# LanaSina/evolutionary_illusion_generator

Measured on AMD Instinct MI355X. Metric: genome fitness evals/sec at 256x256, pop=256, higher is better.
Workload: dtype f32; 1 GPU; neat_configs/circles.txt colour pop=256, 256x256, PredNet 3,48,96,192, 21 steps, LK + rotation-symmetry score; global_pop=256, genomes_per_gpu=256, device_batch=256, structure=Circles

## Files before the change

evolutionary_illusion_generator_amd/csrc/conv_wino4.h:

```cpp
#pragma once
#include "wino_launch.h"

namespace eig {

constexpr int W4_UPOS = 256;
constexpr int W4_U_FLOATS = W4_NPOS * W4_UPOS;
constexpr int W4_NUS = 3, W4_NPS = 3;
constexpr int w4_row(bool tall) { return tall ? 28 : 40; }
constexpr int w4_ps(bool tall) { return tall ? 1024 : 768; }
constexpr int w4_pslot(bool tall) { return W4_KC * w4_ps(tall); }
constexpr int w4_p(bool tall, int k) { return tall ? k * w4_pslot(true) : (k < 2 ? k * w4_pslot(false) : 2 * w4_pslot(false) + 3 * W4_U_FLOATS); }
constexpr int w4_u(bool tall, int k) { return tall ? 3 * w4_pslot(true) + k * W4_U_FLOATS : 2 * w4_pslot(false) + k * W4_U_FLOATS; }
constexpr int w4_x(bool tall) { return tall ? w4_u(true, 0) : w4_u(false, 1); }
constexpr int W4_X_FLOATS = W4_WAVES * 2 * 4 * 64 * 4;
constexpr int wino4_lds_bytes() { return (w4_x(false) + W4_X_FLOATS) * 4; }
static_assert((w4_u(true, 2) + W4_U_FLOATS) * 4 == wino4_lds_bytes() && (w4_p(false, 2) + w4_pslot(false)) * 4 <= wino4_lds_bytes(), "LDS maps");
#ifndef EIG_W4_DEEPU
#define EIG_W4_DEEPU 1
#endif
#ifndef EIG_W4_DIAG
#define EIG_W4_DIAG 0
#endif

__device__ __forceinline__ void w4_in1d(float d0, float d1, float d2, float d3, float d4, float d5, float* T)
{
    T[0] = fmaf(4.0f, d0, fmaf(-5.0f, d2, d4));
    const float p = fmaf(-4.0f, d2, d4), q = fmaf(-4.0f, d1, d3);
    T[1] = p + q; T[2] = p - q;
    const float r = d4 - d2, s = d3 - d1;
    T[3] = fmaf(2.0f, s, r); T[4] = fmaf(-2.0f, s, r);
    T[5] = fmaf(4.0f, d1, fmaf(-5.0f, d3, d5));
}
template <int XI> __device__ __forceinline__ float w4_row(const float* d)
{
    if constexpr (XI == 0) return fmaf(4.0f, d[0], fmaf(-5.0f, d[1], d[2]));
    else if constexpr (XI == 5) return fmaf(4.0f, d[0], fmaf(-5.0f, d[1], d[2]));
    else {
        if constexpr (XI == 1) return fmaf(-4.0f, d[1], d[3]) + fmaf(-4.0f, d[0], d[2]);
        else if constexpr (XI == 2) return fmaf(-4.0f, d[1], d[3]) - fmaf(-4.0f, d[0], d[2]);
        else if constexpr (XI == 3) return fmaf(2.0f, d[2] - d[0], d[3] - d[1]);
        else return fmaf(-2.0f, d[2] - d[0], d[3] - d[1]);
    }
}
constexpr int w4_nrows(int xi) { return (xi == 0 || xi == 5) ? 3 : 4; }
constexpr int w4_rowidx(int xi, int k) { return xi == 0 ? 2 * k : xi == 5 ? 2 * k + 1 : k + 1; }
constexpr int w4_uprow(int i) { return (i + 1) >> 1; }

template <typename V4> __device__ __forceinline__ void w4_out1d(const V4& m0, const V4& m1, const V4& m2, const V4& m3, const V4& m4, const V4& m5, V4* Y)
{
    const V4 s = m1 + m2, d = m1 - m2, u = m3 + m4, w = m3 - m4;
    Y[0] = (m0 + s) + u;
    for (int e = 0; e < 4; ++e) { Y[1][e] = fmaf(2.0f, w[e], d[e]); Y[2][e] = fmaf(4.0f, u[e], s[e]); Y[3][e] = fmaf(8.0f, w[e], d[e]) + m5[e]; }
}

template <int NI, int EPI, bool TALL = false, bool HALF = false, bool PACK = false, bool NSPLIT = false>
__global__ void __launch_bounds__((HALF && !NSPLIT) ? W4_THREADS / 2 : W4_THREADS, 3) wino4_kernel(const ConvArgs a)
{
    static_assert(!NSPLIT || (HALF && NI == 4 && EPI != EPI_CONVA), "N-split: a half block, 64-column N-blocks, ConvLSTM / ConvP");
    constexpr int NIW = NSPLIT ? 2 : NI;
    constexpr bool DEEPU = HALF && EIG_W4_DEEPU;
    static_assert(!(TALL && HALF), "half blocks exist in the wide shape only");
    static_assert(!PACK || (HALF && EPI != EPI_CONVA), "packed tiles: a half block, ConvLSTM / ConvP");
    constexpr bool TGEO = TALL || PACK;
    static_assert(EPI == EPI_LSTM || EPI == EPI_CONVA || EPI == EPI_CONVP, "conv_wino4.h: ConvLSTM, ConvA, ConvP");
    static_assert(EPI != EPI_LSTM || NI == 4, "ConvLSTM: the four N-tiles are the four gates");
    static_assert(NI == 3 || NI == 4, "N-blocks of 48 or 64 columns");
    constexpr int U4 = wino4_u_floats(NI);
    constexpr int KC = W4_KC, PS = w4_ps(TGEO), W4_ROW = w4_row(TGEO);
    constexpr int W4_P0 = w4_p(TGEO, 0), W4_P1 = w4_p(TGEO, 1), W4_P2 = w4_p(TGEO, 2), W4_U0 = w4_u(TGEO, 0), W4_U1 = w4_u(TGEO, 1), W4_U2 = w4_u(TGEO, 2);
    constexpr int PK_ROWS = 18, PK_CX = 7, PK_IMG = PK_ROWS * PK_CX;
    constexpr bool WALK = !TALL && !HALF;
    constexpr int RGH = TALL ? 16 : 8;
    extern __shared__ __attribute__((aligned(16))) float lds[];
    unsigned long long tq_entry = EIG_TIMING ? __builtin_readcyclecounter() : 0;
    float* const Pb = lds;
    float* const Ub = lds;
    float* const xb = lds + w4_x(TGEO);
    const int wv_o = __builtin_amdgcn_readfirstlane((int)threadIdx.x >> 6);
    const int rg_o = HALF ? 0 : wv_o & 1, xi_o = (HALF && !NSPLIT) ? wv_o : wv_o >> 1;
    const int ng_o = NSPLIT ? wv_o & 1 : 0;
    constexpr int NWAVES = (HALF && !NSPLIT) ? W4_WAVES / 2 : W4_WAVES;
    constexpr int UPW = 36 / NWAVES;
    auto lane_id = [&]() __attribute__((always_inline)) { int l = (int)__builtin_amdgcn_mbcnt_hi(~0u, __builtin_amdgcn_mbcnt_lo(~0u, 0u)); asm volatile("" : "+v"(l)); return l; };

    const int tiles = a.tilesX * a.tilesY;
    const bool pk5 = PACK && a.tilesX == 5;
    const int ntile = PACK ? a.B + (pk5 ? (a.B + 3) >> 2 : 0) : a.B * tiles;
    const int xcd = blockIdx.x & 7, xi_ = blockIdx.x >> 3;
    auto dv = [&](int x, int d, unsigned m) __attribute__((always_inline)) { return m ? (int)__umulhi((unsigned)x, m) : x / d; };
    const int q0 = dv(xi_, a.nparts, a.mg[0]);
    const int part = xi_ - q0 * a.nparts;
    const int tlin = a.tile_map ? xcd * ((ntile + 7) >> 3) + q0 : q0 * 8 + xcd;
    if (tlin >= ntile) return;
    const int nwalk = WALK ? a.nwalk : 1, nb0 = part * nwalk;
    const bool pk_edge_o = pk5 && tlin >= a.B;
    const int eb = PACK ? (pk_edge_o ? 4 * (tlin - a.B) : tlin) : dv(tlin, tiles, a.mg[1]);
    const int t_ = PACK ? 0 : tlin - eb * tiles;
    const int tyi = dv(t_, a.tilesX, a.mg[2]), txi = t_ - tyi * a.tilesX;
    const int y0 = PACK ? 0 : tyi * (TALL ? 32 : (HALF ? 8 : 16)), x0 = PACK ? 0 : txi * (TALL ? 16 : 32);
    const int HW = a.H * a.W;

    const bool up_fused = !PACK && EPI == EPI_LSTM && a.up_src != nullptr;
    const int nkb0 = a.src[0].C / KC;
    const int nkbu = up_fused ? (a.up_C / KC) : 0;
    const bool has1 = a.nsrc > 1;
    const int nkb_o = nkb0 + nkbu + (has1 ? (a.src[1].C / KC) : 0);
    const int up_lo_o = nkb0, up_hi_o = nkb0 + nkbu;
#define EIG4_WAITCNT(imm) do { __builtin_amdgcn_s_waitcnt(imm); asm volatile("" ::: "memory"); } while (0)
#define EIG4_BARRIER() do { asm volatile("" ::: "memory"); __builtin_amdgcn_s_barrier(); asm volatile("" ::: "memory"); } while (0)
#define EIG4_LDS_BARRIER() do { EIG4_WAITCNT(0xC07F); EIG4_BARRIER(); } while (0)
#define EIG4_IS_UP(kb) ((kb) >= up_lo && (kb) < up_hi)

    typedef float f32x2 __attribute__((ext_vector_type(2)));
    constexpr unsigned W4_POSB = 4 * 16 * NI * 4;
    auto walk_body = [&](const int it) __attribute__((always_inline)) {
    const int nblk = nb0 + it;
    int zs = 0;
    asm volatile("" : "+s"(zs));
    const int wv = wv_o + zs, rg = rg_o + zs, xi = xi_o + zs, ng = ng_o + zs, nkb = nkb_o + zs, up_lo = up_lo_o + zs, up_hi = up_hi_o + zs;
    const int pch = HALF ? wv >> 1 : wv / 3, ppart = HALF ? wv & 1 : wv - pch * 3;
    const bool has_plane = !(NSPLIT && !PACK) || wv_o < 8;
    const int eb_i = eb + zs, y0_i = y0 + zs, x0_i = x0 + zs;
    const bool pk_edge = (pk_edge_o ? 1 : 0) + zs != 0;
    const unsigned long long sb0 = (unsigned long long)(a.src[0].ptr + (size_t)eb_i * a.src[0].Ct * HW);
    const unsigned long long sb1 = has1 ? (unsigned long long)(a.src[1].ptr + (size_t)eb_i * a.src[1].Ct * HW) : sb0;
    const int ist0 = a.src[0].Ct * HW * 4, ist1 = has1 ? a.src[1].Ct * HW * 4 : ist0;
    const int sz0 = a.src[0].C * HW * 4 + (PACK ? 3 * ist0 : 0), sz1 = has1 ? a.src[1].C * HW * 4 + (PACK ? 3 * ist1 : 0) : sz0;
    const int Hh = a.H >> 1, Wh = a.W >> 1, HWh = Hh * Wh;
    const unsigned long long sbu = up_fused ? (unsigned long long)(a.up_src + (size_t)eb_i * a.up_C * HWh) : sb0;
    const int szu = up_fused ? a.up_C * HWh * 4 : sz0;
    const int lane = lane_id();
    const int q = lane >> 4, col = lane & 15;
    constexpr int CPR = TALL ? 7 : 10, CREAL = TALL ? 6 : 10, NCHK = TALL ? 34 * 7 : (HALF ? 100 : 180), UROWS = TALL ? 18 : (HALF ? 6 : 10), UCHK = TALL ? 4 : 6;
    auto plane_offsets = [&](int part, int& ro, int& uo) __attribute__((always_inline)) {
        const int c = lane + 64 * part;
        const int row = c / CPR, cx = c - row * CPR;
        const int gy = y0_i - 1 + row, gx = x0_i - 4 + 4 * cx;
        ro = (c < NCHK && cx < CREAL && gy >= 0 && gy < a.H && gx >= 0 && gx < a.W) ? (gy * a.W + gx) * 4 : -1;
        const int hy = (y0_i >> 1) - 1 + row, hx = (x0_i >> 1) - 4 + 4 * cx;
        uo = (row < UROWS && cx < UCHK && hy >= 0 && hy < Hh && hx >= 0 && hx < Wh) ? (hy * Wh + hx) * 4 : -1;
    };
    int pk_ro[3] = {-1, -1, -1};
    unsigned pk_mul[3] = {0u, 0u, 0u};
    const int pk_n = (wv_o < 4 ? 2 : 1) + (NSPLIT ? 0 : 1);
    if constexpr (PACK) {
#pragma unroll
        for (int k = 0; k < 3; ++k) {
            const int c = lane + 64 * ((wv_o + NWAVES * k) & 3);
            const int p = c >= PK_IMG ? 1 : 0, c1 = c - PK_IMG * p;
            const int row = c1 / PK_CX, slot = c1 - row * PK_CX;
            const int b = slot >= 3 ? (slot >= 6 ? 2 : 1) : 0;
            const int irel = pk_edge ? 2 * p + b : 0, cx = pk_edge ? 4 + slot - 3 * b : slot;
            const int gy = row - 1, gx = 4 * cx - 4;
            const bool ok = (pk_edge ? (c < 2 * PK_IMG && b < 2) : c < PK_IMG) && eb_i + irel < a.B && gy >= 0 && gy < a.H && gx >= 0 && gx < a.W;
            pk_ro[k] = ok ? (gy * a.W + gx) * 4 : -1;
            pk_mul[k] = ok ? (unsigned)irel : 0u;
        }
    }
    int roff, uoff, roff2 = -1, uoff2 = -1;
    plane_offsets(ppart, roff, uoff);
    const bool two_parts = (TALL && wv_o < 4) || (HALF && !PACK && !NSPLIT && wv_o < 2);
    if (TALL) plane_offsets(3, roff2, uoff2);
    if (HALF) { roff2 = roff; uoff2 = uoff; }
    const int ch2 = HALF ? 3 : wv, part2 = HALF ? ppart : 3;
    auto dma_plane_at = [&](int jj, int slot_off) __attribute__((always_inline)) {
        const int j = jj < nkb ? jj : nkb - 1;
        const bool up = EIG4_IS_UP(j);
        const bool s1 = j >= up_hi;
        const unsigned long long mu = 0ull - (unsigned long long)up, m1 = 0ull - (unsigned long long)s1;
        const unsigned long long u = sb0 + ((sb1 - sb0) & m1) + ((sbu - sb0) & mu);
        const unsigned lo = __builtin_amdgcn_readfirstlane((unsigned)u), hi = __builtin_amdgcn_readfirstlane((unsigned)(u >> 32));
        const int sz = sz0 + ((sz1 - sz0) & (int)m1) + ((szu - sz0) & (int)mu);
        const __amdgpu_buffer_rsrc_t rs = __builtin_amdgcn_make_buffer_rsrc((void*)(((unsigned long long)hi << 32) | lo), 0, __builtin_amdgcn_readfirstlane(sz), 0x00020000);
        const int base = (up_lo & (int)mu) + (up_hi & (int)m1), hw = HW + ((HWh - HW) & (int)mu);
        if constexpr (PACK) {
            const unsigned ist = (unsigned)(ist0 + ((ist1 - ist0) & (int)m1));
#pragma unroll
            for (int k = 0; k < 3; ++k) {
                if (k >= pk_n) break;
                const int idx = wv_o + NWAVES * k;
                const unsigned coffk = (unsigned)((j - base) * KC + (idx >> 2)) * (unsigned)(hw * 4);
                __builtin_amdgcn_raw_ptr_buffer_load_lds(rs, (__attribute__((address_space(3))) void*)(Pb + slot_off + (idx >> 2) * PS + (idx & 3) * 256), 16,
                                                         (int)__builtin_elementwise_add_sat((unsigned)pk_ro[k] + pk_mul[k] * ist, coffk), 0, 0, 0);
            }
            return;
        }
        if (!has_plane) return;
        const unsigned coff = (unsigned)((j - base) * KC + pch) * (unsigned)(hw * 4);
        __builtin_amdgcn_raw_ptr_buffer_load_lds(rs, (__attribute__((address_space(3))) void*)(Pb + slot_off + pch * PS + ppart * 256), 16,
                                                 (int)__builtin_elementwise_add_sat((unsigned)roff + (((unsigned)uoff - (unsigned)roff) & (unsigned)mu), coff), 0, 0, 0);
        if (two_parts) {
            const unsigned coff2 = (unsigned)((j - base) * KC + ch2) * (unsigned)(hw * 4);
            __builtin_amdgcn_raw_ptr_buffer_load_lds(rs, (__attribute__((address_space(3))) void*)(Pb + slot_off + ch2 * PS + part2 * 256), 16,
                                                     (int)__builtin_elementwise_add_sat((unsigned)roff2 + (((unsigned)uoff2 - (unsigned)roff2) & (unsigned)mu), coff2), 0, 0, 0);
        }
    };
    auto wait_u = [&]() __attribute__((always_inline)) {
        const int npl = PACK ? pk_n : (two_parts ? 2 : (has_plane ? 1 : 0));
        switch (npl + (DEEPU ? UPW : 0)) {
            case 0: EIG4_WAITCNT(0x0F70); break;
            case 1: EIG4_WAITCNT(0x0F71); break;
            case 2: EIG4_WAITCNT(0x0F72); break;
            case 3: EIG4_WAITCNT(0x0F73); break;
            case 4: EIG4_WAITCNT(0x0F74); break;
            case 5: EIG4_WAITCNT(0x0F75); break;
            case 6: EIG4_WAITCNT(0x0F76); break;
            case 7: EIG4_WAITCNT(0x0F77); break;
            case 8: EIG4_WAITCNT(0x0F78); break;
            default: EIG4_WAITCNT(0x0F79); break;
        }
    };
    const int uvo = (NI == 4 || lane < 48) ? lane * 16 : -1;
    auto prologue_a = [&](int nb) __attribute__((always_inline)) {
        const __amdgpu_buffer_rsrc_t rs = __builtin_amdgcn_make_buffer_rsrc((void*)(a.wpk + (size_t)nb * nkb * U4), 0, (nkb + 1) * U4 * 4, 0x00020000);
#pragma unroll
        for (int i = 0; i < UPW; ++i)
            __builtin_amdgcn_raw_ptr_buffer_load_lds(rs, (__attribute__((address_space(3))) void*)(Ub + W4_U0 + (UPW * wv + i) * W4_UPOS), 16, uvo, (int)((unsigned)(UPW * wv + i) * W4_POSB), 0, 0);
        dma_plane_at(0, W4_P0);
        dma_plane_at(1, W4_P1);
    };
    auto prologue_b = [&](int nb) __attribute__((always_inline)) {
        const __amdgpu_buffer_rsrc_t rs = __builtin_amdgcn_make_buffer_rsrc((void*)(a.wpk + (size_t)nb * nkb * U4), 0, (nkb + 1) * U4 * 4, 0x00020000);
#pragma unroll
        for (int i = 0; i < UPW; ++i)
            __builtin_amdgcn_raw_ptr_buffer_load_lds(rs, (__attribute__((address_space(3))) void*)(Ub + W4_U1 + (UPW * wv + i) * W4_UPOS), 16, uvo,
                                                     (int)((unsigned)U4 * 4 + (unsigned)(UPW * wv + i) * W4_POSB), 0, 0);
        dma_plane_at(2, W4_P2);
    };

    const int pk_ir = pk_edge ? col >> 2 : 0, pk_ty = pk_edge ? col & 3 : col >> 2;
    const int t_ty = PACK ? 0 : (TALL ? col >> 2 : col >> 3), t_tx = PACK ? (pk_edge ? 3 * (pk_ir & 1) : col & 3) : (TALL ? col & 3 : col & 7);
    const int pk_row = PACK ? PK_ROWS * (pk_ir >> 1) + 4 * pk_ty : 0;
    const float* const pbase_n = Pb + q * PS + (RGH * rg + 4 * t_ty + pk_row) * W4_ROW + 4 * t_tx;
    const float* const pbase_u = Pb + q * PS + ((RGH / 2) * rg + 2 * t_ty) * W4_ROW + 2 * t_tx + 3;
    const int b_off = xi * 6 * W4_UPOS + (q * 16 + col) * NI + 2 * ng;

    unsigned long long tq_setup = tq_entry;
    if (it == 0) {
        if (EIG_TIMING) tq_setup = __builtin_readcyclecounter();
        prologue_a(nb0);
        EIG4_WAITCNT(0x0F70);
    }
    const __amdgpu_buffer_rsrc_t rsw = __builtin_amdgcn_make_buffer_rsrc((void*)(a.wpk + (size_t)nblk * nkb * U4), 0, (nkb + 1) * U4 * 4, 0x00020000);
    unsigned u_so = (unsigned)(UPW * wv) * W4_POSB + 2u * (unsigned)U4 * 4u;
    auto dma_u = [&](int slot_off) __attribute__((always_inline)) {
#pragma unroll
        for (int i = 0; i < UPW; ++i)
            __builtin_amdgcn_raw_ptr_buffer_load_lds(rsw, (__attribute__((address_space(3))) void*)(Ub + slot_off + (UPW * wv + i) * W4_UPOS), 16, uvo,
                                                     (int)(u_so + (unsigned)i * W4_POSB), 0, 0);
        u_so += (unsigned)U4 * 4;
    };
    f32x4 acc[6][NIW];
#pragma unroll
    for (int p = 0; p < 6; ++p)
#pragma unroll
        for (int ni = 0; ni < NIW; ++ni) acc[p][ni] = (f32x4){0.f, 0.f, 0.f, 0.f};
    EIG4_BARRIER();
    prologue_b(nblk);
    const unsigned long long tq_k0 = EIG_TIMING ? __builtin_readcyclecounter() : 0;
    unsigned long long tq_k1 = 0, tq_x = 0, tq_y = 0;
    auto timeline = [&]() __attribute__((always_inline)) {
        if (EIG_TIMING && a.dbg && lane_id() == 0) {
            unsigned hwid, xcc;
            asm volatile("s_getreg_b32 %0, hwreg(HW_REG_HW_ID)" : "=s"(hwid));
            asm volatile("s_getreg_b32 %0, hwreg(HW_REG_XCC_ID)" : "=s"(xcc));
            unsigned long long* dd = a.dbg + (((size_t)blockIdx.x * nwalk + it) * NWAVES + wv) * 8;
            const unsigned long long tq_end = __builtin_readcyclecounter();
            dd[0] = tq_entry; dd[1] = tq_setup; dd[2] = tq_k0; dd[3] = tq_k1; dd[4] = tq_x; dd[5] = tq_y; dd[6] = tq_end;
            dd[7] = (unsigned long long)hwid | ((unsigned long long)xcc << 32);
            tq_entry = tq_end;
        }
    };

    auto kloops = [&](auto role_tag) __attribute__((always_inline)) {
        constexpr int XI = decltype(role_tag)::value;
        float v[6];
        float bq[NIW];
        int uo0 = W4_U0, uo1 = W4_U1, uo2 = W4_U2;
        int po0 = W4_P0, po1 = W4_P1, po2 = W4_P2;
        int pj = 0, psz = 0, pbound = 0;
        unsigned pcoff = 0, plo = 0, phi = 0, phw4 = 0, pist = 0;
        bool pup = false;
        auto plane_source = [&](int j) __attribute__((always_inline)) {
            const bool up = EIG4_IS_UP(j);
            const bool s1 = j >= up_hi;
            const unsigned long long mu = 0ull - (unsigned long long)up, m1 = 0ull - (unsigned long long)s1;
            const unsigned long long u = sb0 + ((sb1 - sb0) & m1) + ((sbu - sb0) & mu);
            plo = __builtin_amdgcn_readfirstlane((unsigned)u); phi = __builtin_amdgcn_readfirstlane((unsigned)(u >> 32));
            psz = __builtin_amdgcn_readfirstlane(sz0 + ((sz1 - sz0) & (int)m1) + ((szu - sz0) & (int)mu));
            const int base = (up_lo & (int)mu) + (up_hi & (int)m1);
            phw4 = (unsigned)((HW + ((HWh - HW) & (int)mu)) * 4);
            pcoff = (unsigned)((j - base) * KC + (PACK ? 0 : pch)) * phw4;
            if constexpr (PACK) pist = (unsigned)(ist0 + ((ist1 - ist0) & (int)m1));
            pup = up; pj = j;
            pbound = j < up_lo ? up_lo : (j < up_hi ? up_hi : nkb);
        };
        auto dma_plane = [&]() __attribute__((always_inline)) {
            const unsigned o = (unsigned)roff + (((unsigned)uoff - (unsigned)roff) & (0u - (unsigned)pup));
            const __amdgpu_buffer_rsrc_t prs = __builtin_amdgcn_make_buffer_rsrc((void*)(((unsigned long long)phi << 32) | plo), 0, psz, 0x00020000);
            if constexpr (PACK) {
#pragma unroll
                for (int k = 0; k < 3; ++k) {
                    if (k >= pk_n) break;
                    const int idx = wv + NWAVES * k;
                    __builtin_amdgcn_raw_ptr_buffer_load_lds(prs, (__attribute__((address_space(3))) void*)(Pb + po0 + (idx >> 2) * PS + (idx & 3) * 256), 16,
                                                             (int)__builtin_elementwise_add_sat((unsigned)pk_ro[k] + pk_mul[k] * pist, pcoff + (unsigned)(idx >> 2) * phw4), 0, 0, 0);
                }
            } else if (has_plane) {
            __builtin_amdgcn_raw_ptr_buffer_load_lds(prs, (__attribute__((address_space(3))) void*)(Pb + po0 + pch * PS + ppart * 256), 16,
                                                     (int)__builtin_elementwise_add_sat(o, pcoff), 0, 0, 0);
            }
            if (two_parts) {
                const unsigned o2 = (unsigned)roff2 + (((unsigned)uoff2 - (unsigned)roff2) & (0u - (unsigned)pup));
                __builtin_amdgcn_raw_ptr_buffer_load_lds(prs, (__attribute__((address_space(3))) void*)(Pb + po0 + ch2 * PS + part2 * 256), 16,
                                                         (int)__builtin_elementwise_add_sat(o2, pcoff + (unsigned)(ch2 - pch) * phw4), 0, 0, 0);
            }
            if (__builtin_expect(pj + 1 == pbound, 0)) { if (pbound < nkb) plane_source(pj + 1); }
            else { ++pj; pcoff += KC * phw4; }
        };
        plane_source(3 < nkb ? 3 : nkb - 1);
        float pr[2][6];
        float t[6];
        int rso = 0;
        bool rup = false;
        auto read_rows = [&](int ph) __attribute__((always_inline)) {
            if (EIG_W4_DIAG & 4) return;
            constexpr bool END = XI == 0 || XI == 5;
#pragma unroll
            for (int j = 0; j < 2; ++j) {
                const int k = ph == 0 ? (END ? 1 + j : 1 + 2 * j) : (END ? 0 : 2 * j);
                if (ph == 1 && END && j == 1) continue;
                if (rup) {
                    const float* const pl = pbase_u + rso + w4_uprow(w4_rowidx(XI, k)) * W4_ROW;
                    const float s0 = pl[0], s1_ = pl[1], s2 = pl[2], s3 = pl[3];
                    pr[j][0] = s0; pr[j][1] = s1_; pr[j][2] = s1_; pr[j][3] = s2; pr[j][4] = s2; pr[j][5] = s3;
                } else {
                    const float* const pl = pbase_n + rso + w4_rowidx(XI, k) * W4_ROW;
                    typedef const volatile __attribute__((address_space(3))) f32x2* lds_f32x2;
                    const f32x2 c0 = *(lds_f32x2)(pl + 2), c2 = *(lds_f32x2)(pl + 8);
                    const f32x4 c1 = *reinterpret_cast<const f32x4*>(pl + 4);
                    pr[j][0] = c0[1]; pr[j][1] = c1[0]; pr[j][2] = c1[1]; pr[j][3] = c1[2]; pr[j][4] = c1[3]; pr[j][5] = c2[0];
                }
            }
        };
        auto rows_begin = [&](int slot_off, bool up) __attribute__((always_inline)) {
            rso = slot_off; rup = up;
            read_rows(0);
        };
        auto rows_mid = [&]() __attribute__((always_inline)) {
            if (!(EIG_W4_DIAG & 4)) {
#pragma unroll
                for (int c = 0; c < 6; ++c) {
                    if constexpr (XI == 0 || XI == 5) t[c] = fmaf(-5.0f, pr[0][c], pr[1][c]);
                    else if constexpr (XI == 1 || XI == 2) t[c] = fmaf(-4.0f, pr[0][c], pr[1][c]);
                    else t[c] = pr[1][c] - pr[0][c];
                }
            }
            read_rows(1);
        };
        auto rows_end = [&]() __attribute__((always_inline)) {
            if (EIG_W4_DIAG & 4) return;
#pragma unroll
            for (int c = 0; c < 6; ++c) {
                if constexpr (XI == 0 || XI == 5) t[c] = fmaf(4.0f, pr[0][c], t[c]);
                else if constexpr (XI == 1) t[c] = t[c] + fmaf(-4.0f, pr[0][c], pr[1][c]);
                else if constexpr (XI == 2) t[c] = t[c] - fmaf(-4.0f, pr[0][c], pr[1][c]);
                else if constexpr (XI == 3) t[c] = fmaf(2.0f, pr[1][c] - pr[0][c], t[c]);
                else t[c] = fmaf(-2.0f, pr[1][c] - pr[0][c], t[c]);
            }
        };
        auto build_cols = [&]() __attribute__((always_inline)) {
            if (EIG_W4_DIAG & 4) { for (int c = 0; c < 6; ++c) v[c] = 1.0f; return; }
            w4_in1d(t[0], t[1], t[2], t[3], t[4], t[5], v);
        };
        auto read_b = [&](int slot_off, int nu, float* dst) __attribute__((always_inline)) {
            const float* const bsrc = Ub + slot_off + b_off + nu * W4_UPOS;
            if constexpr (NSPLIT) {
                const f32x2 b2 = *reinterpret_cast<const f32x2*>(bsrc);
                dst[0] = b2[0]; dst[1] = b2[1];
            } else if constexpr (NI == 4) {
                const f32x4 b4 = *reinterpret_cast<const f32x4*>(bsrc);
                dst[0] = b4[0]; dst[1] = b4[1]; dst[2] = b4[2]; dst[3] = b4[3];
            } else {
#pragma unroll
                for (int ni = 0; ni < NI; ++ni) dst[ni] = bsrc[ni];
            }
        };
        auto kiter = [&](const int kb, auto kind_tag, auto nk_tag, auto last_tag, auto first_tag) __attribute__((always_inline)) {
            constexpr int KIND = decltype(kind_tag)::value;
            constexpr int NK = decltype(nk_tag)::value;
            constexpr bool LAST = decltype(last_tag)::value;
            constexpr bool FIRST = decltype(first_tag)::value || (DEEPU && !LAST);
            constexpr bool UP = KIND == 1;
            constexpr bool IDLE = UP && XI == 2;
            constexpr int NCH = IDLE ? 0 : (UP ? 5 : 6);
            float bv[2][NIW];
            auto slice = [&](int i) __attribute__((always_inline)) {
                if constexpr (!LAST) {
                    if (i == 0) { if (!(EIG_W4_DIAG & 16)) dma_u(uo2); }
                    if (i == 1) { if (!(EIG_W4_DIAG & 8)) dma_plane(); }
                    if (i == NCH - 4) rows_begin(po1, NK == 2 ? EIG4_IS_UP(kb + 1) : NK == 1);
                    if (i == NCH - 3) rows_mid();
                    if (i == NCH - 2) rows_end();
                    if (i == NCH - 1) build_cols();
                }
            };
            if constexpr (IDLE) {
                if constexpr (!LAST) {
                    if (!(EIG_W4_DIAG & 16)) dma_u(uo2);
                    if (!(EIG_W4_DIAG & 8)) dma_plane();
                    rows_begin(po1, NK == 2 ? EIG4_IS_UP(kb + 1) : NK == 1); rows_mid(); rows_end();
                    if constexpr (!FIRST) read_b(uo1, 0, bq);
                    build_cols();
                }
            } else {
#pragma unroll
                for (int i = 0; i < NCH; ++i) {
                    const int nu = (UP && i >= 2) ? i + 1 : i;
                    if (i + 1 < NCH) {
                        const int nu1 = (UP && i + 1 >= 2) ? i + 2 : i + 1;
                        read_b(uo0, nu1, bv[(i + 1) & 1]);
                    } else if constexpr (!LAST && !FIRST) read_b(uo1, 0, bq);
                    const float* const b = i == 0 ? bq : bv[i & 1];
#pragma unroll
                    for (int ni = 0; ni < NIW; ++ni) acc[nu][ni] = __builtin_amdgcn_mfma_f32_16x16x4f32(v[nu], b[ni], acc[nu][ni], 0, 0, 0);
                    slice(i);
                    __builtin_amdgcn_sched_barrier(0);
                }
            }
            { const int t0 = uo0; uo0 = uo1; uo1 = uo2; uo2 = t0; }
            { const int t0 = po0; po0 = po1; po1 = po2; po2 = t0; }
            if (LAST || (EIG_W4_DIAG & (8 | 16))) EIG4_WAITCNT(0x0F70);
            else if (!(EIG_W4_DIAG & 2)) { if (!(EIG_W4_DIAG & 1)) wait_u(); }
            if (!(EIG_W4_DIAG & 2) || LAST) EIG4_BARRIER();
            if constexpr (FIRST) read_b(uo0, 0, bq);
        };
        const std::false_type nl{};
        const std::integral_constant<int, 2> rt{};
        int kb = 0;
        rows_begin(W4_P0, EIG4_IS_UP(0)); rows_mid(); rows_end();
        read_b(W4_U0, 0, bq);
        build_cols();
        EIG4_WAITCNT(0xC07F);
        EIG4_BARRIER();
        auto run = [&](const int end, auto kind_tag) __attribute__((always_inline)) {
            for (; kb + 1 < end; ++kb) kiter(kb, kind_tag, kind_tag, nl, nl);
            if (kb + 1 == end && end < nkb) { kiter(kb, kind_tag, rt, nl, nl); ++kb; }
        };
        kiter(0, std::integral_constant<int, 0>{}, std::integral_constant<int, 0>{}, nl, std::true_type{});
        kb = 1;
        run(up_lo, std::integral_constant<int, 0>{});
        run(up_hi, std::integral_constant<int, 1>{});
        run(nkb, std::integral_constant<int, 0>{});
        kiter(nkb - 1, rt, rt, std::true_type{}, nl);
    };
    switch (xi) {
        case 0: kloops(std::integral_constant<int, 0>{}); break;
        case 1: kloops(std::integral_constant<int, 1>{}); break;
        case 2: kloops(std::integral_constant<int, 2>{}); break;
        case 3: kloops(std::integral_constant<int, 3>{}); break;
        case 4: kloops(std::integral_constant<int, 4>{}); break;
        default: kloops(std::integral_constant<int, 5>{}); break;
    }
    if (EIG_TIMING) tq_k1 = __builtin_readcyclecounter();
    const bool more = it + 1 < nwalk;
    if (more) prologue_a(nblk + 1);

    f32x4 cc[4][NIW];
#pragma unroll
    for (int ni = 0; ni < NIW; ++ni) {
        f32x4 Y[4];
        w4_out1d(acc[0][ni], acc[1][ni], acc[2][ni], acc[3][ni], acc[4][ni], acc[5][ni], Y);
#pragma unroll
        for (int b = 0; b < 4; ++b) cc[b][ni] = Y[b];
    }
    {
    int zf = 0;
    asm volatile("" : "+s"(zf));
    const int eb = eb_i + zf, y0 = y0_i + zf, x0 = x0_i + zf, wv = wv_o + zf, rg = rg_o + zf, xi = xi_o + zf, HWf = HW + zf, Cout = a.Cout + zf, ngf = ng_o + zf;
    const bool pk_edge_f = (pk_edge_o ? 1 : 0) + zf != 0;
    const int lane = lane_id();
    const int q = lane >> 4, col = lane & 15;
    const size_t cHW = (size_t)HWf;
    const int j = TALL ? lane & 3 : lane & 7, chl = TALL ? lane >> 2 : lane >> 3, e_r = j & 3, ql = TALL ? 0 : j >> 2;
    int woff[4];
#pragma unroll
    for (int e = 0; e < 4; ++e) woff[e] = (((2 * xi + (NSPLIT ? ngf : rg)) * 2 * 4 + e) * 64 + q * 16 + ((col + 4 * e + (PACK ? q : (TALL ? 0 : 8 * (q & 1)))) & 15)) * 4;
    const int fr = lane & 15, fchl = lane >> 4;
    const int f_i = pk_edge_f ? fr >> 2 : 0, f_ty = pk_edge_f ? fr & 3 : fr >> 2, f_tx = pk_edge_f ? 4 : fr & 3;
    if constexpr (EPI == EPI_LSTM || EPI == EPI_CONVP) {
        const int nun = NSPLIT ? ((xi < 4 && ngf == 0) ? 2 : 1) : (xi < 4 ? 3 : 2);
        auto unit_cq = [&](int un) __attribute__((always_inline)) { return xi < 4 ? (NSPLIT ? (ngf ? 2 : un) : un) : 3; };
        auto unit_arow = [&](int un) __attribute__((always_inline)) { return xi < 4 ? xi : 2 * (xi - 4) + (NSPLIT ? ngf : un); };
        int xoff[3];
#pragma unroll
        for (int un = 0; un < 3; ++un) {
            const int cq = unit_cq(un);
            const int ty = TALL ? cq : cq >> 1, chh = TALL ? 0 : cq & 1;
            xoff[un] = TALL ? (e_r * 64 + ty * 16 + ((chl + 4 * e_r) & 15)) * 4 : (e_r * 64 + (2 * ty + ql) * 16 + ((8 * chh + chl + 4 * e_r + 8 * ql) & 15)) * 4;
            if constexpr (PACK) xoff[un] = ((fr & 3) * 64 + (fr >> 2) * 16 + ((4 * cq + fchl + 4 * (fr & 3) + (fr >> 2)) & 15)) * 4;
        }
        auto finish = [&](int arow, int nr, int off, int xw) __attribute__((always_inline)) -> f32x4 {
            auto C = [&](int x) __attribute__((always_inline)) { return *reinterpret_cast<const f32x4*>(xb + ((x * 2 + xw) * 2 + nr) * 1024 + off); };
            const f32x4 c1 = C(1), c2 = C(2), c3 = C(3), c4 = C(4);
            const f32x4 s_ = c1 + c2, d_ = c1 - c2, u_ = c3 + c4, w_ = c3 - c4;
            f32x4 y;
            if (arow == 0) { const f32x4 c0 = C(0); y = (c0 + s_) + u_; }
            else if (arow == 1) { for (int b = 0; b < 4; ++b) y[b] = fmaf(2.0f, w_[b], d_[b]); }
            else if (arow == 2) { for (int b = 0; b < 4; ++b) y[b] = fmaf(4.0f, u_[b], s_[b]); }
            else { const f32x4 c5 = C(5); for (int b = 0; b < 4; ++b) y[b] = fmaf(8.0f, w_[b], d_[b]) + c5[b]; }
            return y;
        };
        f32x4 ys[NI][3];
        auto finish_unit = [&](int ni, int nr, int xw, int un) __attribute__((always_inline)) {
            const int sel = NSPLIT ? ngf : un;
            switch (xi) {
                case 0: ys[ni][un] = finish(0, nr, xoff[un], xw); break;
                case 1: ys[ni][un] = finish(1, nr, xoff[un], xw); break;
                case 2: ys[ni][un] = finish(2, nr, xoff[un], xw); break;
                case 3: ys[ni][un] = finish(3, nr, xoff[un], xw); break;
                case 4: ys[ni][un] = sel ? finish(1, nr, xoff[un], xw) : finish(0, nr, xoff[un], xw); break;
                default: ys[ni][un] = sel ? finish(3, nr, xoff[un], xw) : finish(2, nr, xoff[un], xw); break;
            }
        };
        if constexpr (NSPLIT) {
#pragma unroll
            for (int nr = 0; nr < 2; ++nr)
#pragma unroll
                for (int e = 0; e < 4; ++e) {
                    f32x4 t;
                    t[0] = cc[0][nr][e]; t[1] = cc[1][nr][e]; t[2] = cc[2][nr][e]; t[3] = cc[3][nr][e];
                    *reinterpret_cast<f32x4*>(xb + woff[e] + nr * 1024) = t;
                }
            EIG4_LDS_BARRIER();
            if (EIG_TIMING) tq_x = __builtin_readcyclecounter();
#pragma unroll
            for (int ni = 0; ni < NI; ++ni)
#pragma unroll
                for (int un = 0; un < 2; ++un) {
                    if (un >= nun) break;
                    finish_unit(ni, ni & 1, ni >> 1, un);
                }
        } else {
#pragma unroll
        for (int rnd = 0; rnd < 2; ++rnd) {
            if (2 * rnd >= NI) break;
            if (rnd) EIG4_LDS_BARRIER();
#pragma unroll
            for (int nr = 0; nr < 2; ++nr) {
                const int ni = 2 * rnd + nr;
                if (ni >= NI) break;
#pragma unroll
                for (int e = 0; e < 4; ++e) {
                    f32x4 t;
                    t[0] = cc[0][ni][e]; t[1] = cc[1][ni][e]; t[2] = cc[2][ni][e]; t[3] = cc[3][ni][e];
                    *reinterpret_cast<f32x4*>(xb + woff[e] + nr * 1024) = t;
                }
            }
            EIG4_LDS_BARRIER();
            if (EIG_TIMING && rnd == 0) tq_x = __builtin_readcyclecounter();
#pragma unroll
            for (int nr = 0; nr < 2; ++nr) {
                const int ni = 2 * rnd + nr;
                if (ni >= NI) break;
#pragma unroll
                for (int un = 0; un < 3; ++un) {
                    if (un >= nun) break;
                    finish_unit(ni, nr, rg, un);
                }
            }
        }
        }
        if (more) EIG4_WAITCNT(0x0F70);
        if (EIG_TIMING) { asm volatile("s_waitcnt lgkmcnt(0)" ::: "memory"); tq_y = __builtin_readcyclecounter(); }
#pragma unroll
        for (int un = 0; un < 3; ++un) {
            if (un >= nun) break;
            const int cq = unit_cq(un);
            const int ty = TALL ? cq : cq >> 1, chh = TALL ? 0 : cq & 1;
            const int arow = unit_arow(un);
            const int gy = PACK ? 4 * f_ty + arow : y0 + RGH * rg + 4 * ty + arow, gx = PACK ? 4 * f_tx : x0 + 4 * j;
            if (gy >= a.H || gx >= a.W) continue;
            const int ebo = PACK ? eb + f_i : eb;
            if (PACK && ebo >= a.B) continue;
            const size_t pix = (size_t)gy * a.W + gx;
            const int chq = PACK ? 4 * cq + fchl : 8 * chh + chl;
            if constexpr (EPI == EPI_LSTM) {
                const int ch = nblk * 16 + chq;
                if (ch >= Cout) continue;
                const float bi = a.bias[ch], bf = a.bias[Cout + ch], bc = a.bias[2 * Cout + ch], bo = a.bias[3 * Cout + ch];
                const size_t cbase = ((size_t)ebo * Cout + ch) * cHW, ps = (size_t)Cout * cHW, pbase = (size_t)ch * cHW;
                const f32x4 cold4 = *reinterpret_cast<const f32x4*>(a.c_state + cbase + pix);
                const f32x4 pi4 = *reinterpret_cast<const f32x4*>(a.peep + pbase + pix);
                const f32x4 pf4 = *reinterpret_cast<const f32x4*>(a.peep + ps + pbase + pix);
                const f32x4 po4 = *reinterpret_cast<const f32x4*>(a.peep + 2 * ps + pbase + pix);
                f32x4 cn4, hn4;
#pragma unroll
                for (int b = 0; b < 4; ++b) {
                    float cn, hn;
                    lstm_cell(ys[0][un][b], ys[1][un][b], ys[2][un][b], ys[3][un][b], bi, bf, bc, bo, cold4[b], pi4[b], pf4[b], po4[b], cn, hn);
                    cn4[b] = cn; hn4[b] = hn;
                }
                *reinterpret_cast<f32x4*>(a.c_state + cbase + pix) = cn4;
                *reinterpret_cast<f32x4*>(a.h_out + cbase + pix) = hn4;
            } else {
#pragma unroll
                for (int ni = 0; ni < NI; ++ni) {
                    const int ch = (nblk * NI + ni) * 16 + chq;
                    if (ch >= Cout) continue;
                    const float bb_ = a.bias[ch];
                    f32x4 v4;
#pragma unroll
                    for (int b = 0; b < 4; ++b) v4[b] = relu_f(ys[ni][un][b] + bb_);
                    *reinterpret_cast<f32x4*>(a.Pout + ((size_t)ebo * Cout + ch) * cHW + pix) = v4;
                }
            }
        }
    } else {
        const int Ho = a.H >> 1, Wo = a.W >> 1;
        const size_t plane = (size_t)Ho * Wo;
        const int ox = (x0 >> 1) + 2 * j;
#pragma unroll
        for (int rnd = 0; rnd < 2; ++rnd) {
            if (2 * rnd >= NI) break;
            const int nval = NI - 2 * rnd >= 2 ? 2 : 1;
            if (rnd) EIG4_LDS_BARRIER();
#pragma unroll
            for (int nr = 0; nr < 2; ++nr) {
                if (nr >= nval) break;
                const int ni = 2 * rnd + nr;
#pragma unroll
                for (int e = 0; e < 4; ++e) {
                    f32x4 t;
                    t[0] = cc[0][ni][e]; t[1] = cc[1][ni][e]; t[2] = cc[2][ni][e]; t[3] = cc[3][ni][e];
                    *reinterpret_cast<f32x4*>(xb + woff[e] + nr * 1024) = t;
                }
            }
            EIG4_LDS_BARRIER();
            if (rnd == (NI - 1) / 2) { if (more) EIG4_WAITCNT(0x0F70); }
            if (EIG_TIMING && rnd == 0) { tq_x = __builtin_readcyclecounter(); tq_y = tq_x; }
            const int g0 = nval == 2 ? (xi < 4 ? 3 * xi : 12 + 2 * (xi - 4)) : (xi < 2 ? 2 * xi : xi + 2);
            const int cnt = nval == 2 ? (xi < 4 ? 3 : 2) : (xi < 2 ? 2 : 1);
#pragma unroll
            for (int un = 0; un < 3; ++un) {
                if (un >= cnt) break;
                const int g = g0 + un;
                const int nr = g >> 3, ty = TALL ? (g >> 1) & 3 : (g >> 2) & 1, ap = TALL ? g & 1 : (g >> 1) & 1, chh = TALL ? 0 : g & 1;
                const int off = TALL ? ((nr + 2 * rg) * 256 + e_r * 64 + ty * 16 + ((chl + 4 * e_r) & 15)) * 4
                                     : ((nr + 2 * rg) * 256 + e_r * 64 + (2 * ty + ql) * 16 + ((8 * chh + chl + 4 * e_r + 8 * ql) & 15)) * 4;
                auto C = [&](int x) __attribute__((always_inline)) { return *reinterpret_cast<const f32x4*>(xb + x * 4096 + off); };
                const f32x4 c1 = C(1), c2 = C(2), c3 = C(3), c4 = C(4);
                const f32x4 s_ = c1 + c2, d_ = c1 - c2, u_ = c3 + c4, w_ = c3 - c4;
                f32x4 ya, yb;
                if (ap == 0) {
                    const f32x4 c0 = C(0);
                    ya = (c0 + s_) + u_;
                    for (int b = 0; b < 4; ++b) yb[b] = fmaf(2.0f, w_[b], d_[b]);
                } else {
                    const f32x4 c5 = C(5);
                    for (int b = 0; b < 4; ++b) { ya[b] = fmaf(4.0f, u_[b], s_[b]); yb[b] = fmaf(8.0f, w_[b], d_[b]) + c5[b]; }
                }
                const int ch = (nblk * NI + 2 * rnd + nr) * 16 + 8 * chh + chl;
                const int oy = (y0 >> 1) + (RGH / 2) * rg + 2 * ty + ap;
                if (oy >= Ho || ox >= Wo || ch >= Cout) continue;
                const float bb_ = a.bias[ch];
                const size_t pb = ((size_t)eb * Cout + ch) * plane + (size_t)oy * Wo + ox;
                const size_t e0 = ((size_t)eb * 2 * Cout + ch) * plane + (size_t)oy * Wo + ox, e1 = e0 + (size_t)Cout * plane;
                const f32x2 p2 = *reinterpret_cast<const f32x2*>(a.P + pb);
                f32x2 ea, eb2;
#pragma unroll
                for (int bp = 0; bp < 2; ++bp) {
                    const float v00 = relu_f(ya[2 * bp] + bb_), v01 = relu_f(ya[2 * bp + 1] + bb_);
                    const float v10 = relu_f(yb[2 * bp] + bb_), v11 = relu_f(yb[2 * bp + 1] + bb_);
                    const float A = fmaxf(fmaxf(v00, v01), fmaxf(v10, v11));
                    ea[bp] = relu_f(A - p2[bp]);
                    eb2[bp] = relu_f(p2[bp] - A);
                }
                *reinterpret_cast<f32x2*>(a.E + e0) = ea;
                *reinterpret_cast<f32x2*>(a.E + e1) = eb2;
            }
        }
    }
    }
    timeline();
    };
    for (int it = 0; it < nwalk; ++it) walk_body(it);
#undef EIG4_WAITCNT
#undef EIG4_BARRIER
#undef EIG4_LDS_BARRIER
#undef EIG4_IS_UP
}

}
```

Baseline: 429.5 genome evals/s.

## Split Winograd k-iteration into head/tail to overlap first MFMA across barrier

Restructures the Winograd-4 K loop so the first channel's MFMAs (head) of the next k-block are issued right after the previous block's barrier, separately from the remaining MFMAs and DMA/row-building slices (tail). The b-fragment buffer is hoisted out of the per-iteration lambda so it can carry across the split, and an empty asm pins the v registers on tall tiles. The plane-source pointer advance is also rewritten so the increment is unconditional with a rare rollback. The aim is to cut MFMA idle time around the barrier and wait, at the cost of more complex control flow and possible register pressure or scheduling regressions.

```diff
diff --git a/evolutionary_illusion_generator_amd/csrc/conv_wino4.h b/evolutionary_illusion_generator_amd/csrc/conv_wino4.h
--- a/evolutionary_illusion_generator_amd/csrc/conv_wino4.h
+++ b/evolutionary_illusion_generator_amd/csrc/conv_wino4.h
@@ -315,8 +315,11 @@
                 __builtin_amdgcn_raw_ptr_buffer_load_lds(prs, (__attribute__((address_space(3))) void*)(Pb + po0 + ch2 * PS + part2 * 256), 16,
                                                          (int)__builtin_elementwise_add_sat(o2, pcoff + (unsigned)(ch2 - pch) * phw4), 0, 0, 0);
             }
-            if (__builtin_expect(pj + 1 == pbound, 0)) { if (pbound < nkb) plane_source(pj + 1); }
-            else { ++pj; pcoff += KC * phw4; }
+            ++pj; pcoff += KC * phw4;
+            if (__builtin_expect(pj == pbound, 0)) {
+                if (pbound < nkb) plane_source(pj);
+                else { --pj; pcoff -= KC * phw4; }
+            }
         };
         plane_source(3 < nkb ? 3 : nkb - 1);
         float pr[2][6];
@@ -386,7 +389,22 @@
                 for (int ni = 0; ni < NI; ++ni) dst[ni] = bsrc[ni];
             }
         };
-        auto kiter = [&](const int kb, auto kind_tag, auto nk_tag, auto last_tag, auto first_tag) __attribute__((always_inline)) {
+        float bv[2][NIW];
+        auto khead_mfma = [&]() __attribute__((always_inline)) {
+            __builtin_amdgcn_sched_barrier(0);
+            acc[0][0] = __builtin_amdgcn_mfma_f32_16x16x4f32(v[0], bq[0], acc[0][0], 0, 0, 0);
+            __builtin_amdgcn_sched_barrier(0);
+            read_b(uo0, 1, bv[1]);
+#pragma unroll
+            for (int ni = 1; ni < NIW; ++ni) acc[0][ni] = __builtin_amdgcn_mfma_f32_16x16x4f32(v[0], bq[ni], acc[0][ni], 0, 0, 0);
+            __builtin_amdgcn_sched_barrier(0);
+        };
+        auto khead = [&](const int kb, auto kind_tag) __attribute__((always_inline)) {
+            constexpr int KIND = decltype(kind_tag)::value;
+            if constexpr (XI != 2 || KIND == 0) khead_mfma();
+            else if constexpr (KIND == 2) khead_mfma();
+        };
+        auto ktail = [&](const int kb, auto kind_tag, auto nk_tag, auto last_tag, auto first_tag) __attribute__((always_inline)) {
             constexpr int KIND = decltype(kind_tag)::value;
             constexpr int NK = decltype(nk_tag)::value;
             constexpr bool LAST = decltype(last_tag)::value;
@@ -394,7 +412,6 @@
             constexpr bool UP = KIND == 1;
             constexpr bool IDLE = UP && XI == 2;
             constexpr int NCH = IDLE ? 0 : (UP ? 5 : 6);
-            float bv[2][NIW];
             auto slice = [&](int i) __attribute__((always_inline)) {
                 if constexpr (!LAST) {
                     if (i == 0) { if (!(EIG_W4_DIAG & 16)) dma_u(uo2); }
@@ -414,20 +431,23 @@
                     build_cols();
                 }
             } else {
-#pragma unroll
-                for (int i = 0; i < NCH; ++i) {
+                slice(0);
+                __builtin_amdgcn_sched_barrier(0);
+#pragma unroll
+                for (int i = 1; i < NCH; ++i) {
                     const int nu = (UP && i >= 2) ? i + 1 : i;
                     if (i + 1 < NCH) {
                         const int nu1 = (UP && i + 1 >= 2) ? i + 2 : i + 1;
                         read_b(uo0, nu1, bv[(i + 1) & 1]);
                     } else if constexpr (!LAST && !FIRST) read_b(uo1, 0, bq);
-                    const float* const b = i == 0 ? bq : bv[i & 1];
+                    const float* const b = bv[i & 1];
 #pragma unroll
                     for (int ni = 0; ni < NIW; ++ni) acc[nu][ni] = __builtin_amdgcn_mfma_f32_16x16x4f32(v[nu], b[ni], acc[nu][ni], 0, 0, 0);
                     slice(i);
                     __builtin_amdgcn_sched_barrier(0);
                 }
             }
+            if constexpr (TALL && !LAST) asm volatile("" : "+v"(v[0]), "+v"(v[1]), "+v"(v[2]), "+v"(v[3]), "+v"(v[4]), "+v"(v[5]));
             { const int t0 = uo0; uo0 = uo1; uo1 = uo2; uo2 = t0; }
             { const int t0 = po0; po0 = po1; po1 = po2; po2 = t0; }
             if (LAST || (EIG_W4_DIAG & (8 | 16))) EIG4_WAITCNT(0x0F70);
@@ -436,6 +456,7 @@
             if constexpr (FIRST) read_b(uo0, 0, bq);
         };
         const std::false_type nl{};
+        const std::integral_constant<int, 0> full{};
         const std::integral_constant<int, 2> rt{};
         int kb = 0;
         rows_begin(W4_P0, EIG4_IS_UP(0)); rows_mid(); rows_end();
@@ -444,15 +465,16 @@
         EIG4_WAITCNT(0xC07F);
         EIG4_BARRIER();
         auto run = [&](const int end, auto kind_tag) __attribute__((always_inline)) {
-            for (; kb + 1 < end; ++kb) kiter(kb, kind_tag, kind_tag, nl, nl);
-            if (kb + 1 == end && end < nkb) { kiter(kb, kind_tag, rt, nl, nl); ++kb; }
-        };
-        kiter(0, std::integral_constant<int, 0>{}, std::integral_constant<int, 0>{}, nl, std::true_type{});
+            const int m = end - (end == nkb ? 1 : 0);
+            for (; kb + 1 < m; ++kb) { ktail(kb, kind_tag, kind_tag, nl, nl); khead(kb + 1, kind_tag); }
+            if (kb + 1 == m) { ktail(kb, kind_tag, rt, nl, nl); ++kb; khead(kb, rt); }
+        };
+        khead(0, full); ktail(0, full, full, nl, std::true_type{}); khead(1, full);
         kb = 1;
-        run(up_lo, std::integral_constant<int, 0>{});
+        run(up_lo, full);
         run(up_hi, std::integral_constant<int, 1>{});
-        run(nkb, std::integral_constant<int, 0>{});
-        kiter(nkb - 1, rt, rt, std::true_type{}, nl);
+        run(nkb, full);
+        ktail(nkb - 1, rt, rt, std::true_type{}, nl);
     };
     switch (xi) {
         case 0: kloops(std::integral_constant<int, 0>{}); break;
```

After: 440.9 genome evals/s, median of 6. +2.7%, better.
